# microsoft/ConfigNet

Hardware: AMD Instinct MI355X
Metric: train-step images/sec at 256x256 (G+D fwd+bwd) (higher is better)
Workload: dtype f32; 1 GPU; ConfigNet second-stage iteration (D + synth-D + latent-D + G + EMA), 256x256, batch 16 per GPU, fp32, Keras-Adam; global_batch=16, resolution=256, latent_dim=145, parallelism=dp1, losses_finite=True

## Files before the change

### confignet_amd/csrc/winograd4.hip

```cpp
#include "common.h"

#include "mma_tile.h"

namespace {

typedef __attribute__((address_space(3))) float lds_float4;
typedef float v2f __attribute__((ext_vector_type(2)));

struct Wino4Geom {
    int n, h, w, cin, cout, bh, bw;
};

__global__ void wino4_filter_kernel(const float* __restrict__ W, float* __restrict__ U, int cin, int cout, int dgrad) {
    const long total = (long)cin * cout;
    for (long e = (long)blockIdx.x * blockDim.x + threadIdx.x; e < total; e += (long)gridDim.x * blockDim.x) {
        const int co = (int)(e % cout), ci = (int)(e / cout);
        float g[3][3];
#pragma unroll
        for (int a = 0; a < 3; ++a)
#pragma unroll
            for (int b = 0; b < 3; ++b)
                g[a][b] = dgrad ? W[((long)((2 - a) * 3 + (2 - b)) * cin + ci) * cout + co] : W[((long)(a * 3 + b) * cin + ci) * cout + co];
        float t[6][3];
#pragma unroll
        for (int b = 0; b < 3; ++b) {
            const float g0 = g[0][b], g1 = g[1][b], g2 = g[2][b];
            t[0][b] = 0.25f * g0;
            t[1][b] = (-1.f / 6.f) * (g0 + g1 + g2);
            t[2][b] = (-1.f / 6.f) * (g0 - g1 + g2);
            t[3][b] = (1.f / 24.f) * g0 + (1.f / 12.f) * g1 + (1.f / 6.f) * g2;
            t[4][b] = (1.f / 24.f) * g0 - (1.f / 12.f) * g1 + (1.f / 6.f) * g2;
            t[5][b] = g2;
        }
        const long k = dgrad ? co : ci, nn = dgrad ? ci : co;
        const long kdim = dgrad ? cout : cin, ndim = dgrad ? cin : cout;
#pragma unroll
        for (int a = 0; a < 6; ++a) {
            const float t0 = t[a][0], t1 = t[a][1], t2 = t[a][2];
            float u[6];
            u[0] = 0.25f * t0;
            u[1] = (-1.f / 6.f) * (t0 + t1 + t2);
            u[2] = (-1.f / 6.f) * (t0 - t1 + t2);
            u[3] = (1.f / 24.f) * t0 + (1.f / 12.f) * t1 + (1.f / 6.f) * t2;
            u[4] = (1.f / 24.f) * t0 - (1.f / 12.f) * t1 + (1.f / 6.f) * t2;
            u[5] = t2;
#pragma unroll
            for (int b = 0; b < 6; ++b) U[((long)(a * 6 + b) * kdim + k) * ndim + nn] = u[b];
        }
    }
}

#ifndef W4_ABLATE
#define W4_ABLATE 0
#endif
constexpr int W4_KC = 4;
constexpr int W4_T = 32;
constexpr int W4_C = 64;
constexpr int W4_VP = 40;
constexpr int W4_U = 36 * W4_KC * W4_C;
constexpr int W4_RAW_PIECES = 21;
constexpr int W4_RAW = W4_RAW_PIECES * 256;
constexpr int W4_BUF = 2 * W4_U + 2 * W4_RAW;


__global__ __launch_bounds__(768) void wino4_fwd_kernel(Wino4Geom g, const float* __restrict__ X, const float* __restrict__ U,
                                                        const float* __restrict__ bias, float* __restrict__ Y, int act, float slope) {
    __shared__ __attribute__((aligned(16))) float Vs[2][36][W4_KC][W4_VP];
    extern __shared__ __attribute__((aligned(16))) float BUF[];
    const int tid = threadIdx.x, lane = tid & 63, wave = __builtin_amdgcn_readfirstlane(tid >> 6);
    const int half = lane >> 5, l31 = lane & 31;
    const int wi = wave % 6, cb = wave / 6;

    const int nblk = g.n * g.bh * g.bw, total = nblk * (g.cout / W4_C);
    int wg = blockIdx.x;
    if (total % 8 == 0) wg = (wg & 7) * (total >> 3) + (wg >> 3);
    const int blk = wg % nblk, co0 = (wg / nblk) * W4_C;
    int img, brem, by, bx;
    divmod_pos(blk, g.bh * g.bw, img, brem);
    divmod_pos(brem, g.bw, by, bx);

    const __amdgpu_buffer_rsrc_t xres = __builtin_amdgcn_make_buffer_rsrc(const_cast<float*>(X), 0, g.n * g.h * g.w * g.cin * 4, 0x00020000);
    const __amdgpu_buffer_rsrc_t ures = __builtin_amdgcn_make_buffer_rsrc(const_cast<float*>(U), 0, 36 * g.cin * g.cout * 4, 0x00020000);

    unsigned uoff[3];
#pragma unroll
    for (int j = 0; j < 3; ++j) {
        const int p = wave + 12 * j;
        uoff[j] = (unsigned)((p * g.cin + (lane >> 4)) * g.cout + co0 + (lane & 15) * 4) * 4u;
    }
    unsigned xoff[2];
#pragma unroll
    for (int j = 0; j < 2; ++j) {
        const int q = wave + 12 * j, sl = (q * 64 + lane) >> 1;
        const int r = sl / 36, rem = sl - r * 36, cm = rem / 9, c = (rem - cm * 9) * 4 + cm;
        const int yy = by * 16 - 1 + r, xx = bx * 32 - 1 + c;
        const bool in = q < W4_RAW_PIECES && r < 18 && c < 34 && yy >= 0 && yy < g.h && xx >= 0 && xx < g.w;
        xoff[j] = in ? (unsigned)(((img * g.h + yy) * g.w + xx) * g.cin + (((lane & 1) ^ (r >> 2)) & 1) * 4) * 4u : 0x80000000u;
    }
    auto issue_u = [&](int s) {
        float* dst = BUF + (s & 1) * W4_U;
#pragma unroll
        for (int j = 0; j < 3; ++j)
            __builtin_amdgcn_raw_ptr_buffer_load_lds(ures, (lds_float4*)(dst + (wave + 12 * j) * 256), 16, uoff[j], s * W4_KC * g.cout * 4, 0, 0);
    };
    auto issue_raw = [&](int a) {
        float* dst = BUF + 2 * W4_U + (a & 1) * W4_RAW;
#pragma unroll
        for (int j = 0; j < 2; ++j)
            if (wave + 12 * j < W4_RAW_PIECES)
                __builtin_amdgcn_raw_ptr_buffer_load_lds(xres, (lds_float4*)(dst + (wave + 12 * j) * 256), 16, xoff[j], a * 8 * 4, 0, 0);
    };

    const unsigned buf0 = (unsigned)(unsigned long long)(lds_float4*)BUF;

    const int tk = lane & 3, txl = (lane >> 2) & 3, tyl = (lane >> 4) & 1, txh = lane >> 5;
    const int ttx = txl + 4 * txh, tty = 2 * (wave / 6) + tyl, tt = txl + 4 * tyl + 8 * txh + 16 * (wave / 6);
    int trow[4];
    float tco[4];
    {
        const int i = wi;
        trow[0] = i == 0 ? 0 : 1;
        trow[1] = i == 0 ? 2 : (i == 5 ? 3 : 2);
        trow[2] = i == 0 ? 4 : (i == 5 ? 5 : 3);
        trow[3] = 4;
        tco[0] = i == 0 ? 4.f : i == 1 ? -4.f : i == 2 ? 4.f : i == 3 ? -2.f : i == 4 ? 2.f : 4.f;
        tco[1] = i == 0 ? -5.f : i == 1 ? -4.f : i == 2 ? -4.f : i == 3 ? -1.f : i == 4 ? -1.f : -5.f;
        tco[2] = i == 0 ? 1.f : i == 1 ? 1.f : i == 2 ? -1.f : i == 3 ? 2.f : i == 4 ? -2.f : 1.f;
        tco[3] = (i == 0 || i == 5) ? 0.f : 1.f;
    }
    unsigned rbase[4], rsw[4];
#pragma unroll
    for (int q = 0; q < 4; ++q) {
        const int r = 4 * tty + trow[q];
        rbase[q] = buf0 + 4u * (unsigned)(2 * W4_U) + 32u * (unsigned)(r * 36 + ttx) + 4u * (unsigned)tk;
        rsw[q] = (unsigned)((r >> 2) & 1) << 4;
    }
#define W4_RD(q, j, dst) asm volatile("ds_read_b32 %0, %1 offset:%2" : "=v"(dst) : "v"(ra[q]), "i"((((j) & 3) * 9 + ((j) >> 2)) * 32))
    auto transform = [&](int s) {
        const unsigned so = 4u * (unsigned)(((s >> 1) & 1) * W4_RAW), sub = (unsigned)(s & 1) << 4;
        unsigned ra[4];
#pragma unroll
        for (int q = 0; q < 4; ++q) ra[q] = rbase[q] + so + (sub ^ rsw[q]);
        float d[6][4], t[6];
#define W4_COL(c) W4_RD(0, c, d[c][0]); W4_RD(1, c, d[c][1]); W4_RD(2, c, d[c][2]); W4_RD(3, c, d[c][3]);
#define W4_WAIT(pending) asm volatile("s_waitcnt lgkmcnt(" #pending ")"); __builtin_amdgcn_sched_barrier(0);
#define W4_RED(j0, j1)                                                                                                         \
        t[j0] = tco[0] * d[j0][0] + tco[1] * d[j0][1] + tco[2] * d[j0][2] + tco[3] * d[j0][3];                                 \
        t[j1] = tco[0] * d[j1][0] + tco[1] * d[j1][1] + tco[2] * d[j1][2] + tco[3] * d[j1][3];                                 \
        __builtin_amdgcn_sched_barrier(0);
        W4_COL(0) W4_COL(1) W4_COL(2)
        W4_WAIT(4)
        W4_COL(3) W4_COL(4)
        __builtin_amdgcn_sched_barrier(0);
        W4_RED(0, 1)
        W4_WAIT(4)
        W4_COL(5)
        __builtin_amdgcn_sched_barrier(0);
        W4_RED(2, 3)
        W4_WAIT(0)
        W4_RED(4, 5)
#undef W4_WAIT
#undef W4_RED
#undef W4_COL
        float* vdst = &Vs[s & 1][wi * 6][tk][tt];
        constexpr int VPL = W4_KC * W4_VP;
        vdst[0 * VPL] = 4.f * t[0] - 5.f * t[2] + t[4];
        vdst[1 * VPL] = -4.f * (t[1] + t[2]) + t[3] + t[4];
        vdst[2 * VPL] = 4.f * (t[1] - t[2]) - t[3] + t[4];
        vdst[3 * VPL] = -2.f * t[1] - t[2] + 2.f * t[3] + t[4];
        vdst[4 * VPL] = 2.f * t[1] - t[2] - 2.f * t[3] + t[4];
        vdst[5 * VPL] = 4.f * t[1] - 5.f * t[3] + t[5];
    };

    f32x16 acc[6];
#pragma unroll
    for (int j = 0; j < 6; ++j)
#pragma unroll
        for (int r = 0; r < 16; ++r) acc[j][r] = 0.f;

#define W4_RDU(j, kk, dst) asm volatile("ds_read_b32 %0, %1 offset:%2" : "=v"(dst) : "v"(ub), "i"((((j) * W4_KC + 2 * (kk)) * W4_C) * 4))
#define W4_RDA(j, kk, dst) asm volatile("ds_read_b32 %0, %1 offset:%2" : "=v"(dst) : "v"(vb), "i"((((j) * W4_KC + 2 * (kk)) * W4_VP) * 4))
    const unsigned ubase = buf0 + 4u * (unsigned)((wi * 6 * W4_KC + half) * W4_C + cb * 32 + l31);
    const unsigned vbase = (unsigned)(unsigned long long)(lds_float4*)&Vs[0][wi * 6][half][l31];
    auto multiply = [&](int s) {
        const unsigned ub = ubase + 4u * (unsigned)((s & 1) * W4_U);
        const unsigned vb = vbase + 4u * (unsigned)((s & 1) * 36 * W4_KC * W4_VP);
        float a[2][6], b[2][6];
#define W4_PAIR(j, kk) W4_RDA(j, kk, a[kk][j]); W4_RDU(j, kk, b[kk][j]);
#define W4_MFMA(j, kk)                                                                                                         \
        if (!(W4_ABLATE & 1)) acc[j] = __builtin_amdgcn_mfma_f32_32x32x2f32(a[kk][j], b[kk][j], acc[j], 0, 0, 0);              \
        else acc[j][0] += a[kk][j] * b[kk][j];                                                                                 \
        __builtin_amdgcn_sched_barrier(0);
#define W4_WAIT(pending) asm volatile("s_waitcnt lgkmcnt(" #pending ")"); __builtin_amdgcn_sched_barrier(0);
        W4_PAIR(0, 0) W4_PAIR(1, 0) W4_PAIR(2, 0) W4_PAIR(3, 0) W4_PAIR(4, 0) W4_PAIR(5, 0) W4_PAIR(0, 1)
        W4_WAIT(12) W4_MFMA(0, 0) W4_PAIR(1, 1)
        W4_WAIT(12) W4_MFMA(1, 0) W4_PAIR(2, 1)
        W4_WAIT(12) W4_MFMA(2, 0) W4_PAIR(3, 1)
        W4_WAIT(12) W4_MFMA(3, 0) W4_PAIR(4, 1)
        W4_WAIT(12) W4_MFMA(4, 0) W4_PAIR(5, 1)
        W4_WAIT(12) W4_MFMA(5, 0)
        W4_WAIT(10) W4_MFMA(0, 1)
        W4_WAIT(8) W4_MFMA(1, 1)
        W4_WAIT(6) W4_MFMA(2, 1)
        W4_WAIT(4) W4_MFMA(3, 1)
        W4_WAIT(2) W4_MFMA(4, 1)
        W4_WAIT(0) W4_MFMA(5, 1)
#undef W4_WAIT
#undef W4_MFMA
#undef W4_PAIR
    };

    const int nks = (W4_ABLATE & 16) ? 1 : g.cin / W4_KC, nraw = g.cin / 8;
    issue_raw(0);
    issue_u(0);
    __builtin_amdgcn_s_waitcnt(0x0F70);
    __syncthreads();
    if (nraw > 1) issue_raw(1);
    if (nks > 1) issue_u(1);
    transform(0);
    const bool mul_first = ((wave >> 2) & 1) == 0;
    for (int s = 0; s < nks; ++s) {
        __builtin_amdgcn_s_waitcnt(0x0F70);
        __syncthreads();
        if (s >= 1 && !(W4_ABLATE & 4)) {
            if (s + 1 < nks) issue_u(s + 1);
            if ((s & 1) && (s + 3) / 2 < nraw) issue_raw((s + 3) / 2);
        }
#pragma nounroll
        for (int ph = 0; ph < 2; ++ph) {
            if ((ph == 0) == mul_first) multiply(s);
            else if (s + 1 < nks && !(W4_ABLATE & 2)) transform(s + 1);
        }
    }
    __builtin_amdgcn_s_waitcnt(0x0F70);
    __syncthreads();

    float* E = BUF;
    if (W4_ABLATE & 8) {
        float t = 0.f;
#pragma unroll
        for (int j = 0; j < 6; ++j)
#pragma unroll
            for (int r = 0; r < 16; ++r) t += acc[j][r];
        if (t == 12345.f) Y[tid] = t;
        return;
    }
    for (int rb = 0; rb < 2; ++rb) {
        if (cb == rb) {
#pragma unroll
            for (int e = 0; e < 16; ++e) {
                const int tl = 4 * half + (e & 3) + 8 * (e >> 2);
                const float a0 = acc[0][e], a1 = acc[1][e], a2 = acc[2][e], a3 = acc[3][e], a4 = acc[4][e], a5 = acc[5][e];
                const float s12 = a1 + a2, d12 = a1 - a2, s34 = a3 + a4, d34 = a3 - a4;
                float* dst = E + ((wi * 4) * 32 + tl) * 32 + l31;
                dst[0 * 1024] = a0 + s12 + s34;
                dst[1 * 1024] = d12 + 2.f * d34;
                dst[2 * 1024] = s12 + 4.f * s34;
                dst[3 * 1024] = d12 + 8.f * d34 + a5;
            }
        }
        __syncthreads();
        for (int idx = tid; idx < 1024; idx += 768) {
            const int c4 = idx & 7, tl = (idx >> 3) & 31, y = idx >> 8;
            float4 m[6];
#pragma unroll
            for (int i = 0; i < 6; ++i) m[i] = *reinterpret_cast<const float4*>(E + ((i * 4 + y) * 32 + tl) * 32 + 4 * c4);
            const int co = co0 + rb * 32 + 4 * c4;
            const float4 bv = bias ? *reinterpret_cast<const float4*>(bias + co) : make_float4(0.f, 0.f, 0.f, 0.f);
            const int otx = (tl & 3) + 4 * ((tl >> 3) & 1), oty = ((tl >> 2) & 1) + 2 * (tl >> 4);
            const int row0 = by * 16 + 4 * oty, col = bx * 32 + 4 * otx + y;
#define W4_O(f)                                                                                                          \
            const float s12##f = m[1].f + m[2].f, d12##f = m[1].f - m[2].f, s34##f = m[3].f + m[4].f, d34##f = m[3].f - m[4].f; \
            const float o0##f = m[0].f + s12##f + s34##f + bv.f, o1##f = d12##f + 2.f * d34##f + bv.f,                     \
                        o2##f = s12##f + 4.f * s34##f + bv.f, o3##f = d12##f + 8.f * d34##f + m[5].f + bv.f;
            W4_O(x) W4_O(y) W4_O(z) W4_O(w)
#undef W4_O
            float* dst = Y + ((long)(img * g.h + row0) * g.w + col) * g.cout + co;
            const long rs = (long)g.w * g.cout;
            *reinterpret_cast<float4*>(dst) = make_float4(cn_apply_act(o0x, act, slope), cn_apply_act(o0y, act, slope), cn_apply_act(o0z, act, slope), cn_apply_act(o0w, act, slope));
            *reinterpret_cast<float4*>(dst + rs) = make_float4(cn_apply_act(o1x, act, slope), cn_apply_act(o1y, act, slope), cn_apply_act(o1z, act, slope), cn_apply_act(o1w, act, slope));
            *reinterpret_cast<float4*>(dst + 2 * rs) = make_float4(cn_apply_act(o2x, act, slope), cn_apply_act(o2y, act, slope), cn_apply_act(o2z, act, slope), cn_apply_act(o2w, act, slope));
            *reinterpret_cast<float4*>(dst + 3 * rs) = make_float4(cn_apply_act(o3x, act, slope), cn_apply_act(o3y, act, slope), cn_apply_act(o3z, act, slope), cn_apply_act(o3w, act, slope));
        }
        __syncthreads();
    }
}

}

extern "C" int cn_conv_wino4_filter(const float* w, float* u, int cin, int cout, int dgrad, void* stream) {
    CN_CHECK_ARG(w && u && cin > 0 && cout > 0, "wino4_filter: bad args");
    const long total = (long)cin * cout;
    const int blocks = (int)((total + 255) / 256 > 4096 ? 4096 : (total + 255) / 256);
    hipLaunchKernelGGL(wino4_filter_kernel, dim3(blocks), dim3(256), 0, (hipStream_t)stream, w, u, cin, cout, dgrad);
    CN_LAUNCH_CHECK();
    return CN_OK;
}

extern "C" int cn_conv_fwd_wino4(int n, int h, int w, int cin, int cout, const float* x, const float* u, const float* bias,
                                 float* y, int act, float slope, void* stream) {
    CN_CHECK_ARG(x && u && y && n > 0 && h > 0 && w > 0, "conv_fwd_wino4: bad args");
    if (h % 16 || w % 32 || cin % 16 || cout % W4_C) return CN_EUNSUPPORTED;
    CN_CHECK_ARG((double)n * h * w * (cin > cout ? cin : cout) * 4.0 < 2147483647.0 && 144.0 * cin * cout < 2147483647.0,
                 "tensor exceeds 2^31 bytes (buffer descriptors, 32-bit offsets)");
    Wino4Geom g{n, h, w, cin, cout, h / 16, w / 32};
    const long nblk = (long)n * g.bh * g.bw;
    constexpr size_t lds = sizeof(float) * W4_BUF;
    static bool attr_set = false;
    if (!attr_set) {
        CN_HIP(hipFuncSetAttribute(reinterpret_cast<const void*>(wino4_fwd_kernel), hipFuncAttributeMaxDynamicSharedMemorySize, (int)lds));
        attr_set = true;
    }
    hipStream_t s = (hipStream_t)stream;
    cn_prof_begin(s, 2.0 * 36.0 * (double)nblk * W4_T * cin * cout, 4.0 * ((double)n * h * w * (cin + cout) + 36.0 * cin * cout), CN_FAM_WINO);
    hipLaunchKernelGGL(wino4_fwd_kernel, dim3((unsigned)(nblk * (cout / W4_C))), dim3(768), lds, s, g, x, u, bias, y, act, slope);
    cn_prof_end(s);
    CN_LAUNCH_CHECK();
    return CN_OK;
}
```

Baseline: 420.8 images/sec.

## Load Winograd filter tiles directly into registers with MFMA-ready layout, K-chunk 8

Repacks the transformed filter U into a blocked layout matching the MFMA B-operand lane order. The forward kernel then streams it with buffer_load_dwordx2 straight into registers, double-buffered across K steps, instead of staging it through LDS. The K chunk doubles to 8 so there are half as many barriers, and the V tile moves into the dynamic LDS buffer. The aim is to cut LDS traffic and synchronisation in the main loop. The cost is more register pressure, tightly hand-tuned vmcnt waits, and a new layout requirement on cin/cout.

```diff
diff --git a/confignet_amd/csrc/winograd4.hip b/confignet_amd/csrc/winograd4.hip
--- a/confignet_amd/csrc/winograd4.hip
+++ b/confignet_amd/csrc/winograd4.hip
@@ -6,6 +6,7 @@
 
 typedef __attribute__((address_space(3))) float lds_float4;
 typedef float v2f __attribute__((ext_vector_type(2)));
+typedef int v4i __attribute__((ext_vector_type(4)));
 
 struct Wino4Geom {
     int n, h, w, cin, cout, bh, bw;
@@ -33,7 +34,8 @@
             t[5][b] = g2;
         }
         const long k = dgrad ? co : ci, nn = dgrad ? ci : co;
-        const long kdim = dgrad ? cout : cin, ndim = dgrad ? cin : cout;
+        const long kdim = dgrad ? cout : cin;
+        float* ub = U + ((((nn >> 6) * (kdim >> 2) + (k >> 2)) * 36 * 2 + (k & 1)) * 64 + (nn & 63)) * 2 + ((k >> 1) & 1);
 #pragma unroll
         for (int a = 0; a < 6; ++a) {
             const float t0 = t[a][0], t1 = t[a][1], t2 = t[a][2];
@@ -45,7 +47,7 @@
             u[4] = (1.f / 24.f) * t0 - (1.f / 12.f) * t1 + (1.f / 6.f) * t2;
             u[5] = t2;
 #pragma unroll
-            for (int b = 0; b < 6; ++b) U[((long)(a * 6 + b) * kdim + k) * ndim + nn] = u[b];
+            for (int b = 0; b < 6; ++b) ub[(a * 6 + b) * 256] = u[b];
         }
     }
 }
@@ -53,19 +55,20 @@
 #ifndef W4_ABLATE
 #define W4_ABLATE 0
 #endif
-constexpr int W4_KC = 4;
+constexpr int W4_KC = 8;
 constexpr int W4_T = 32;
 constexpr int W4_C = 64;
 constexpr int W4_VP = 40;
-constexpr int W4_U = 36 * W4_KC * W4_C;
+constexpr int W4_V = 36 * W4_KC * W4_VP;
 constexpr int W4_RAW_PIECES = 21;
-constexpr int W4_RAW = W4_RAW_PIECES * 256;
-constexpr int W4_BUF = 2 * W4_U + 2 * W4_RAW;
+constexpr int W4_RAW = 24 * 256;
+constexpr int W4_BUF = 2 * W4_V + 2 * W4_RAW;
+constexpr int W4_UH = 36 * 256 * 4;
+constexpr bool W4_LD = !(W4_ABLATE & 4);
 
 
 __global__ __launch_bounds__(768) void wino4_fwd_kernel(Wino4Geom g, const float* __restrict__ X, const float* __restrict__ U,
                                                         const float* __restrict__ bias, float* __restrict__ Y, int act, float slope) {
-    __shared__ __attribute__((aligned(16))) float Vs[2][36][W4_KC][W4_VP];
     extern __shared__ __attribute__((aligned(16))) float BUF[];
     const int tid = threadIdx.x, lane = tid & 63, wave = __builtin_amdgcn_readfirstlane(tid >> 6);
     const int half = lane >> 5, l31 = lane & 31;
@@ -80,14 +83,15 @@
     divmod_pos(brem, g.bw, by, bx);
 
     const __amdgpu_buffer_rsrc_t xres = __builtin_amdgcn_make_buffer_rsrc(const_cast<float*>(X), 0, g.n * g.h * g.w * g.cin * 4, 0x00020000);
-    const __amdgpu_buffer_rsrc_t ures = __builtin_amdgcn_make_buffer_rsrc(const_cast<float*>(U), 0, 36 * g.cin * g.cout * 4, 0x00020000);
-
-    unsigned uoff[3];
-#pragma unroll
-    for (int j = 0; j < 3; ++j) {
-        const int p = wave + 12 * j;
-        uoff[j] = (unsigned)((p * g.cin + (lane >> 4)) * g.cout + co0 + (lane & 15) * 4) * 4u;
-    }
+    const unsigned long long uaddr = (unsigned long long)U;
+    const v4i ures = {(int)(unsigned)uaddr, (int)((uaddr >> 32) & 0xffffu), 36 * g.cin * g.cout * 4, 0x00020000};
+
+    const unsigned bvoff = (unsigned)((((co0 / W4_C) * (g.cin >> 2) * 36 + 6 * wi) * 256 + half * 128 + (cb * 32 + l31) * 2) * 4);
+    v2f B[2][6];
+#define W4_LDB(h, j, so)                                                                                                        \
+    asm volatile("buffer_load_dwordx2 %0, %1, %2, %3 offen offset:%4" : "=v"(B[h][j])                                            \
+                 : "v"(bvoff), "s"(ures), "s"((so) + ((j) >= 4 ? 4096 : 0)), "i"(((j) & 3) * 1024))
+
     unsigned xoff[2];
 #pragma unroll
     for (int j = 0; j < 2; ++j) {
@@ -97,18 +101,11 @@
         const bool in = q < W4_RAW_PIECES && r < 18 && c < 34 && yy >= 0 && yy < g.h && xx >= 0 && xx < g.w;
         xoff[j] = in ? (unsigned)(((img * g.h + yy) * g.w + xx) * g.cin + (((lane & 1) ^ (r >> 2)) & 1) * 4) * 4u : 0x80000000u;
     }
-    auto issue_u = [&](int s) {
-        float* dst = BUF + (s & 1) * W4_U;
-#pragma unroll
-        for (int j = 0; j < 3; ++j)
-            __builtin_amdgcn_raw_ptr_buffer_load_lds(ures, (lds_float4*)(dst + (wave + 12 * j) * 256), 16, uoff[j], s * W4_KC * g.cout * 4, 0, 0);
-    };
     auto issue_raw = [&](int a) {
-        float* dst = BUF + 2 * W4_U + (a & 1) * W4_RAW;
+        float* dst = BUF + 2 * W4_V + (a & 1) * W4_RAW;
 #pragma unroll
         for (int j = 0; j < 2; ++j)
-            if (wave + 12 * j < W4_RAW_PIECES)
-                __builtin_amdgcn_raw_ptr_buffer_load_lds(xres, (lds_float4*)(dst + (wave + 12 * j) * 256), 16, xoff[j], a * 8 * 4, 0, 0);
+            __builtin_amdgcn_raw_ptr_buffer_load_lds(xres, (lds_float4*)(dst + (wave + 12 * j) * 256), 16, xoff[j], a * 8 * 4, 0, 0);
     };
 
     const unsigned buf0 = (unsigned)(unsigned long long)(lds_float4*)BUF;
@@ -128,48 +125,49 @@
         tco[2] = i == 0 ? 1.f : i == 1 ? 1.f : i == 2 ? -1.f : i == 3 ? 2.f : i == 4 ? -2.f : 1.f;
         tco[3] = (i == 0 || i == 5) ? 0.f : 1.f;
     }
-    unsigned rbase[4], rsw[4];
-#pragma unroll
-    for (int q = 0; q < 4; ++q) {
-        const int r = 4 * tty + trow[q];
-        rbase[q] = buf0 + 4u * (unsigned)(2 * W4_U) + 32u * (unsigned)(r * 36 + ttx) + 4u * (unsigned)tk;
-        rsw[q] = (unsigned)((r >> 2) & 1) << 4;
-    }
+    unsigned rb[2], rrow[4];
+#pragma unroll
+    for (int x = 0; x < 2; ++x)
+        rb[x] = buf0 + 4u * (unsigned)(2 * W4_V) + 32u * (unsigned)(4 * tty * 36 + ttx) + 4u * (unsigned)tk + 16u * (unsigned)((tyl ^ x) & 1);
+#pragma unroll
+    for (int q = 0; q < 4; ++q) rrow[q] = 32u * 36u * (unsigned)trow[q];
+    const unsigned vdbase = buf0 + 4u * (unsigned)((wi * 6 * W4_KC + tk) * W4_VP + tt);
 #define W4_RD(q, j, dst) asm volatile("ds_read_b32 %0, %1 offset:%2" : "=v"(dst) : "v"(ra[q]), "i"((((j) & 3) * 9 + ((j) >> 2)) * 32))
+#define W4_STV(p, val) asm volatile("ds_write_b32 %0, %1 offset:%2" : : "v"(vd), "v"(val), "i"((p) * W4_KC * W4_VP * 4))
     auto transform = [&](int s) {
-        const unsigned so = 4u * (unsigned)(((s >> 1) & 1) * W4_RAW), sub = (unsigned)(s & 1) << 4;
-        unsigned ra[4];
-#pragma unroll
-        for (int q = 0; q < 4; ++q) ra[q] = rbase[q] + so + (sub ^ rsw[q]);
-        float d[6][4], t[6];
+        const unsigned so = 4u * (unsigned)((s & 1) * W4_RAW);
+        const unsigned vd0 = vdbase + 4u * (unsigned)((s & 1) * W4_V);
+#pragma nounroll
+        for (int sub = 0; sub < 2; ++sub) {
+            unsigned ra[4];
+#pragma unroll
+            for (int q = 0; q < 4; ++q) ra[q] = (((sub ^ (trow[q] >> 2)) & 1) ? rb[1] : rb[0]) + (so + rrow[q]);
+            float d[6][4], t[6];
 #define W4_COL(c) W4_RD(0, c, d[c][0]); W4_RD(1, c, d[c][1]); W4_RD(2, c, d[c][2]); W4_RD(3, c, d[c][3]);
 #define W4_WAIT(pending) asm volatile("s_waitcnt lgkmcnt(" #pending ")"); __builtin_amdgcn_sched_barrier(0);
-#define W4_RED(j0, j1)                                                                                                         \
-        t[j0] = tco[0] * d[j0][0] + tco[1] * d[j0][1] + tco[2] * d[j0][2] + tco[3] * d[j0][3];                                 \
-        t[j1] = tco[0] * d[j1][0] + tco[1] * d[j1][1] + tco[2] * d[j1][2] + tco[3] * d[j1][3];                                 \
-        __builtin_amdgcn_sched_barrier(0);
-        W4_COL(0) W4_COL(1) W4_COL(2)
-        W4_WAIT(4)
-        W4_COL(3) W4_COL(4)
-        __builtin_amdgcn_sched_barrier(0);
-        W4_RED(0, 1)
-        W4_WAIT(4)
-        W4_COL(5)
-        __builtin_amdgcn_sched_barrier(0);
-        W4_RED(2, 3)
-        W4_WAIT(0)
-        W4_RED(4, 5)
+#define W4_RED1(j) t[j] = __builtin_fmaf(tco[3], d[j][3], __builtin_fmaf(tco[2], d[j][2], __builtin_fmaf(tco[0], d[j][0], tco[1] * d[j][1])));
+#define W4_RED(j0, j1) W4_RED1(j0) W4_RED1(j1) __builtin_amdgcn_sched_barrier(0);
+            W4_COL(0) W4_COL(1) W4_COL(2)
+            W4_WAIT(4)
+            W4_RED(0, 1)
+            W4_COL(3) W4_COL(4)
+            W4_WAIT(4)
+            W4_RED(2, 3)
+            W4_COL(5)
+            W4_WAIT(0)
+            W4_RED(4, 5)
 #undef W4_WAIT
 #undef W4_RED
+#undef W4_RED1
 #undef W4_COL
-        float* vdst = &Vs[s & 1][wi * 6][tk][tt];
-        constexpr int VPL = W4_KC * W4_VP;
-        vdst[0 * VPL] = 4.f * t[0] - 5.f * t[2] + t[4];
-        vdst[1 * VPL] = -4.f * (t[1] + t[2]) + t[3] + t[4];
-        vdst[2 * VPL] = 4.f * (t[1] - t[2]) - t[3] + t[4];
-        vdst[3 * VPL] = -2.f * t[1] - t[2] + 2.f * t[3] + t[4];
-        vdst[4 * VPL] = 2.f * t[1] - t[2] - 2.f * t[3] + t[4];
-        vdst[5 * VPL] = 4.f * t[1] - 5.f * t[3] + t[5];
+            const unsigned vd = vd0 + (unsigned)sub * (4u * W4_VP * 4u);
+            W4_STV(0, __builtin_fmaf(t[0], 4.f, -(5.f * t[2])) + t[4]);
+            W4_STV(1, __builtin_fmaf(-4.f, t[1] + t[2], t[3]) + t[4]);
+            W4_STV(2, __builtin_fmaf(t[1] - t[2], 4.f, -t[3]) + t[4]);
+            W4_STV(3, __builtin_fmaf(2.f, t[3], __builtin_fmaf(t[1], -2.f, -t[2])) + t[4]);
+            W4_STV(4, __builtin_fmaf(-2.f, t[3], __builtin_fmaf(t[1], 2.f, -t[2])) + t[4]);
+            W4_STV(5, __builtin_fmaf(t[1], 4.f, -(5.f * t[3])) + t[5]);
+        }
     };
 
     f32x16 acc[6];
@@ -178,62 +176,65 @@
 #pragma unroll
         for (int r = 0; r < 16; ++r) acc[j][r] = 0.f;
 
-#define W4_RDU(j, kk, dst) asm volatile("ds_read_b32 %0, %1 offset:%2" : "=v"(dst) : "v"(ub), "i"((((j) * W4_KC + 2 * (kk)) * W4_C) * 4))
-#define W4_RDA(j, kk, dst) asm volatile("ds_read_b32 %0, %1 offset:%2" : "=v"(dst) : "v"(vb), "i"((((j) * W4_KC + 2 * (kk)) * W4_VP) * 4))
-    const unsigned ubase = buf0 + 4u * (unsigned)((wi * 6 * W4_KC + half) * W4_C + cb * 32 + l31);
-    const unsigned vbase = (unsigned)(unsigned long long)(lds_float4*)&Vs[0][wi * 6][half][l31];
+    const int nks = (W4_ABLATE & 16) ? 1 : g.cin / W4_KC;
+
+#define W4_RDA(n) asm volatile("ds_read_b32 %0, %1 offset:%2" : "=v"(a[n]) : "v"(vb), "i"(((((n) % 6) * W4_KC + 2 * ((n) / 6)) * W4_VP) * 4))
+    const unsigned vbase = buf0 + 4u * (unsigned)((wi * 6 * W4_KC + half) * W4_VP + l31);
+    auto wait_b = [&](int s) {
+        if (!W4_LD) asm volatile("s_waitcnt vmcnt(0)");
+        else if (s + 2 < nks) asm volatile("s_waitcnt vmcnt(8)");
+        else asm volatile("s_waitcnt vmcnt(6)");
+        __builtin_amdgcn_sched_barrier(0);
+    };
     auto multiply = [&](int s) {
-        const unsigned ub = ubase + 4u * (unsigned)((s & 1) * W4_U);
-        const unsigned vb = vbase + 4u * (unsigned)((s & 1) * 36 * W4_KC * W4_VP);
-        float a[2][6], b[2][6];
-#define W4_PAIR(j, kk) W4_RDA(j, kk, a[kk][j]); W4_RDU(j, kk, b[kk][j]);
-#define W4_MFMA(j, kk)                                                                                                         \
-        if (!(W4_ABLATE & 1)) acc[j] = __builtin_amdgcn_mfma_f32_32x32x2f32(a[kk][j], b[kk][j], acc[j], 0, 0, 0);              \
-        else acc[j][0] += a[kk][j] * b[kk][j];                                                                                 \
+        const unsigned vb = vbase + 4u * (unsigned)((s & 1) * W4_V);
+        const int sn = s + 1 < nks ? s + 1 : s;
+        const int so0 = sn * 2 * W4_UH, so1 = so0 + W4_UH;
+        float a[24];
+#define W4_BV(n) ((((n) / 6) & 1) ? B[(n) / 12][(n) % 6].y : B[(n) / 12][(n) % 6].x)
+#define W4_MFMA(n)                                                                                                             \
+        if (!(W4_ABLATE & 1)) acc[(n) % 6] = __builtin_amdgcn_mfma_f32_32x32x2f32(a[n], W4_BV(n), acc[(n) % 6], 0, 0, 0);      \
+        else acc[(n) % 6][0] += a[n] * W4_BV(n);                                                                               \
         __builtin_amdgcn_sched_barrier(0);
 #define W4_WAIT(pending) asm volatile("s_waitcnt lgkmcnt(" #pending ")"); __builtin_amdgcn_sched_barrier(0);
-        W4_PAIR(0, 0) W4_PAIR(1, 0) W4_PAIR(2, 0) W4_PAIR(3, 0) W4_PAIR(4, 0) W4_PAIR(5, 0) W4_PAIR(0, 1)
-        W4_WAIT(12) W4_MFMA(0, 0) W4_PAIR(1, 1)
-        W4_WAIT(12) W4_MFMA(1, 0) W4_PAIR(2, 1)
-        W4_WAIT(12) W4_MFMA(2, 0) W4_PAIR(3, 1)
-        W4_WAIT(12) W4_MFMA(3, 0) W4_PAIR(4, 1)
-        W4_WAIT(12) W4_MFMA(4, 0) W4_PAIR(5, 1)
-        W4_WAIT(12) W4_MFMA(5, 0)
-        W4_WAIT(10) W4_MFMA(0, 1)
-        W4_WAIT(8) W4_MFMA(1, 1)
-        W4_WAIT(6) W4_MFMA(2, 1)
-        W4_WAIT(4) W4_MFMA(3, 1)
-        W4_WAIT(2) W4_MFMA(4, 1)
-        W4_WAIT(0) W4_MFMA(5, 1)
+#define W4_M(n) W4_WAIT(5) W4_MFMA(n) W4_RDA((n) + 6);
+#define W4_ML(n, h, so) W4_WAIT(5) W4_MFMA(n) if (W4_LD) W4_LDB(h, (n) % 6, so); W4_RDA((n) + 6);
+#define W4_MT(n, pending, so) W4_WAIT(pending) W4_MFMA(n) if (W4_LD) W4_LDB(1, (n) % 6, so);
+        W4_RDA(0); W4_RDA(1); W4_RDA(2); W4_RDA(3); W4_RDA(4); W4_RDA(5);
+        wait_b(s);
+        W4_M(0) W4_M(1) W4_M(2) W4_M(3) W4_M(4) W4_M(5)
+        W4_ML(6, 0, so0) W4_ML(7, 0, so0) W4_ML(8, 0, so0) W4_ML(9, 0, so0) W4_ML(10, 0, so0) W4_ML(11, 0, so0)
+        wait_b(s);
+        W4_M(12) W4_M(13) W4_M(14) W4_M(15) W4_M(16) W4_M(17)
+        W4_MT(18, 5, so1) W4_MT(19, 4, so1) W4_MT(20, 3, so1) W4_MT(21, 2, so1) W4_MT(22, 1, so1) W4_MT(23, 0, so1)
+#undef W4_MT
+#undef W4_ML
+#undef W4_M
 #undef W4_WAIT
 #undef W4_MFMA
-#undef W4_PAIR
+#undef W4_BV
     };
 
-    const int nks = (W4_ABLATE & 16) ? 1 : g.cin / W4_KC, nraw = g.cin / 8;
     issue_raw(0);
-    issue_u(0);
-    __builtin_amdgcn_s_waitcnt(0x0F70);
-    __syncthreads();
-    if (nraw > 1) issue_raw(1);
-    if (nks > 1) issue_u(1);
+    issue_raw(1);
+    W4_LDB(0, 0, 0); W4_LDB(0, 1, 0); W4_LDB(0, 2, 0); W4_LDB(0, 3, 0); W4_LDB(0, 4, 0); W4_LDB(0, 5, 0);
+    W4_LDB(1, 0, W4_UH); W4_LDB(1, 1, W4_UH); W4_LDB(1, 2, W4_UH); W4_LDB(1, 3, W4_UH); W4_LDB(1, 4, W4_UH); W4_LDB(1, 5, W4_UH);
+    asm volatile("s_waitcnt vmcnt(14)\n\ts_barrier" ::: "memory");
     transform(0);
     const bool mul_first = ((wave >> 2) & 1) == 0;
     for (int s = 0; s < nks; ++s) {
-        __builtin_amdgcn_s_waitcnt(0x0F70);
-        __syncthreads();
-        if (s >= 1 && !(W4_ABLATE & 4)) {
-            if (s + 1 < nks) issue_u(s + 1);
-            if ((s & 1) && (s + 3) / 2 < nraw) issue_raw((s + 3) / 2);
-        }
+        if (W4_LD) asm volatile("s_waitcnt vmcnt(12) lgkmcnt(0)\n\ts_barrier" ::: "memory");
+        else asm volatile("s_waitcnt vmcnt(0) lgkmcnt(0)\n\ts_barrier" ::: "memory");
+        if (W4_LD && s + 2 < nks) issue_raw(s + 2);
 #pragma nounroll
         for (int ph = 0; ph < 2; ++ph) {
             if ((ph == 0) == mul_first) multiply(s);
             else if (s + 1 < nks && !(W4_ABLATE & 2)) transform(s + 1);
         }
     }
-    __builtin_amdgcn_s_waitcnt(0x0F70);
-    __syncthreads();
+    __builtin_amdgcn_sched_barrier(0);
+    asm volatile("s_waitcnt vmcnt(0) lgkmcnt(0)\n\ts_barrier" ::: "memory");
+    __builtin_amdgcn_sched_barrier(0);
 
     float* E = BUF;
     if (W4_ABLATE & 8) {
@@ -290,6 +291,7 @@
 
 extern "C" int cn_conv_wino4_filter(const float* w, float* u, int cin, int cout, int dgrad, void* stream) {
     CN_CHECK_ARG(w && u && cin > 0 && cout > 0, "wino4_filter: bad args");
+    if ((dgrad ? cout : cin) % 4 || (dgrad ? cin : cout) % W4_C) return CN_EUNSUPPORTED;
     const long total = (long)cin * cout;
     const int blocks = (int)((total + 255) / 256 > 4096 ? 4096 : (total + 255) / 256);
     hipLaunchKernelGGL(wino4_filter_kernel, dim3(blocks), dim3(256), 0, (hipStream_t)stream, w, u, cin, cout, dgrad);
```

Result: faster. 426.0 images/sec, median of 6 (+1.3%).
